# microsoft/fadtk

Measured on AMD Instinct MI355X. Metric: FAD scores/sec + cov-GEMM TFLOP/s (% MFMA peak), N=100k D=512, higher is better.
Workload: dtype f16 in, f16 MFMA with f32 accumulate over <= 8192-row runs, f64 across runs (moments); split-f16 MFMA iterations (f32 accumulate) + exact int8-MFMA products (int32 accumulate) + f64 correction (Frechet)

## Files before the change

fadtk_amd/_capi.py:

```python
from __future__ import annotations

import ctypes as C
import logging
import os
import threading
from pathlib import Path
from typing import Optional, Tuple

import numpy as np

log = logging.getLogger("fadtk_amd")

FAD_OK = 0
FAD_ERR_INVALID = -1
FAD_ERR_NO_DEVICE = -2
FAD_ERR_HIP = -3
FAD_ERR_ALLOC = -4
FAD_ERR_SHAPE = -5
FAD_ERR_TOO_FEW_ROWS = -6
FAD_ERR_NOT_FINITE = -7
FAD_ERR_NOT_CONVERGED = -8

FAD_F16, FAD_BF16, FAD_F32, FAD_F64 = 0, 1, 2, 3
FAD_KAD_GAUSSIAN, FAD_KAD_IQ, FAD_KAD_IMQ = 0, 1, 2
# ... 91 lines not shown
    "fad_moments_set_timing": (C.c_int, [_P, C.c_int]),
    "fad_moments_set_reference_mean": (C.c_int, [_P, C.c_int]),
    "fad_moments_last_timing": (C.c_int, [_P, C.POINTER(C.c_float), C.POINTER(C.c_float), C.POINTER(C.c_int)]),
    "fad_kad_last_plan": (C.c_int, [C.POINTER(_I64)]),
    "fad_stream_create_cu_mask": (C.c_int, [C.c_int, C.POINTER(C.c_uint32), C.c_int, C.POINTER(_P)]),
    "fad_stream_destroy": (C.c_int, [C.c_int, _P]),
    "fad_frechet": (C.c_int, [C.c_int, _P, _P, _P, _P, C.c_double, C.c_int, C.c_double, C.c_int, C.c_int, _P,
                              C.POINTER(C.c_double), C.POINTER(FadDiag)]),
    "fad_frechet_from_moments": (C.c_int, [_P, _P, C.c_int, C.c_double, C.c_int, C.c_double, C.c_int, _P,
                                           C.POINTER(C.c_double), C.POINTER(FadDiag)]),
    "fad_frechet_from_moments_begin": (C.c_int, [_P, _P, C.c_int, C.c_double, C.c_int, _P, C.POINTER(_P)]),
    "fad_frechet_end": (C.c_int, [_P, C.POINTER(C.c_double), C.POINTER(FadDiag)]),
    "fad_frechet_cancel": (C.c_int, [_P]),
    "fad_frechet_from_moments_multi_begin": (C.c_int, [C.c_int, C.POINTER(_P), C.POINTER(_P), C.c_int, C.c_double, C.c_int, _P, C.POINTER(_P)]),
    "fad_frechet_multi_end": (C.c_int, [_P, C.c_int, C.POINTER(C.c_double), C.POINTER(FadDiag)]),
    "fad_frechet_batched_vs_baseline": (C.c_int, [C.c_int, _P, _P, _P, _I64, _I64, C.c_int, C.POINTER(_I64), _I64,
                                                  C.c_int, C.c_int, C.c_int, _P, _P, _P]),
    "fad_resample_num_samples": (_I64, [_I64, C.c_int, C.c_int]),
    "fad_resample_kaiser": (C.c_int, [_P, _I64, C.c_int, C.c_int, C.c_int, _P, _I64, C.c_int, C.c_int, _P]),
    "fad_logmel_vggish_num_examples": (_I64, [_I64]),
    "fad_logmel_vggish": (C.c_int, [_P, C.POINTER(_I64), _I64, _P, _I64, C.POINTER(_I64), C.c_int, C.c_int, _P]),
    "fad_logmel_whisper": (C.c_int, [_P, C.POINTER(_I64), _I64, C.c_int, _P, C.c_int, C.c_int, _P]),
    "fad_logmel_htsat": (C.c_int, [_P, C.POINTER(_I64), _I64, _I64, _P, C.c_int, C.c_int, _P]),
    "fad_kad_median_distance": (C.c_int, [_P, _I64, _I64, _I64, C.c_int, C.c_int, C.POINTER(C.c_double), C.c_int, _P]),
    "fad_kad": (C.c_int, [_P, _I64, _I64, _P, _I64, _I64, _I64, C.c_int, C.c_int, C.c_double, C.POINTER(FadKadResult),
                          C.c_int, _P]),
    "fad_kad_individual": (C.c_int, [_P, _I64, _I64, _P, _I64, _I64, C.POINTER(_I64), _I64, _I64, C.c_int, C.c_int, C.c_double,
                                     C.POINTER(FadKadResult), _P, _P, _P, _P, C.c_int, _P]),
    "fad_kad_uncertainty": (C.c_int, [_P, _I64, _I64, C.POINTER(_P), C.POINTER(_I64), C.POINTER(_I64), C.c_int, _I64, C.c_int, C.c_int,
                                      C.c_double, C.POINTER(FadKadResult), _P, _P, _P, C.c_int, _P]),
# ... 162 lines not shown
```

fadtk_amd/csrc/frechet.hip:

```cpp
#include "frechet_internal.h"
#include "ns_mean.h"
#include "ns_fast.h"
#include "ns_fast_big.h"
#include "ns_fast_res.h"

#include <algorithm>
#include <atomic>
#include <cmath>
#include <type_traits>

namespace fad {

Pool& thread_pool(int device) {
    static thread_local PerThreadDevice<Pool> set;
    return set.get(device);
}
Workspace* free_slot(int device) {
    Pool& p = thread_pool(device);
    for (Workspace& w : p.slot)
        if (!w.busy) { w.pool = &p; return &w; }
    return nullptr;
}

SongKnobs SongKnobs::from_env() {
// ... 650 lines not shown
    const size_t dd = (size_t)d * d, nb = (size_t)d / 32;
    PairBlock b; size_t o = 0;
    auto take = [&](size_t bytes) { const size_t at = o; o += (bytes + 255) & ~(size_t)255; return at; };
    b.hdrA = take(sizeof(nsf::MatHdr)); b.hdrB = take(sizeof(nsf::MatHdr)); b.st = take(sizeof(NsState)); b.s32 = take(sizeof(Ns32State));
    b.partials = take(nb * nb * sizeof(double)); b.stats = take(nsf::kTileStats * nb * nb * sizeof(double));
    b.A64 = take(8 * dd); b.P = take(8 * dd);
    b.Y[0] = take(8 * dd); b.Y[1] = take(8 * dd); b.Z[0] = take(8 * dd); b.Z[1] = take(8 * dd); b.T = take(8 * dd);
    b.digA = take(6 * dd); b.digB = take(6 * dd);
    b.digY[0] = take(6 * dd); b.digYt[0] = take(6 * dd); b.digY[1] = take(6 * dd); b.digYt[1] = take(6 * dd);
    b.mus = take(2 * (size_t)d * sizeof(double)); b.covs = take(2 * dd * sizeof(double));
    b.Rv = take(8 * dd); b.Pv = take(8 * dd); b.Ev = take(8 * dd);
    b.stride = o;
    return b;
}

static int pairs_verify_enqueue(Workspace& ws, int d, int B, hipStream_t st) {
    const size_t dd = (size_t)d * d;
    const PairBlock L = pair_block(d);
    const size_t hs = song_host_stride(d);
    char* blk = static_cast<char*>(ws.fast_pairs.p);
    char* hpin = static_cast<char*>(ws.fast_pairs_pin);
    auto at = [&](size_t off) { return blk + off; };
    auto mat = [&](size_t off) { nsf::SplitMat m; m.a = reinterpret_cast<uint4*>(at(off)); m.at = reinterpret_cast<uint4*>(at(off + 4 * dd)); return m; };
    nsf::SplitArgs g;
    memset(&g, 0, sizeof(g));
    g.d = d; g.gen = ws.multi.gen; g.hA = reinterpret_cast<nsf::MatHdr*>(at(L.hdrA)); g.hB = reinterpret_cast<nsf::MatHdr*>(at(L.hdrB));
    g.pstride = (int64_t)L.stride; g.astride = (int64_t)L.stride;
    g.st = reinterpret_cast<NsState*>(at(L.st)); g.s32 = reinterpret_cast<Ns32State*>(at(L.s32));
    const nsf::SplitMat Y[2] = {mat(L.Y[0]), mat(L.Y[1])}, Z[2] = {mat(L.Z[0]), mat(L.Z[1])};
    const int nb = d / 32;
    int* h_words = reinterpret_cast<int*>(hpin + (nsf::kHostVals + (size_t)(nsf::kTileStats + 2) * nb * nb) * sizeof(double));
    double* h_vstats = reinterpret_cast<double*>(hpin + host_vstats_off(d));
    for (int b = 0; b < B; ++b) reinterpret_cast<int*>(reinterpret_cast<char*>(h_words) + (size_t)b * hs)[13] = 0;
    fast_verify_launch(d, (unsigned)B, g, Y, Z, mat(L.Rv), mat(L.Pv), mat(L.Ev), g.s32, h_vstats, h_words, (int64_t)hs, st);
    FAD_HIP_TRY(hipGetLastError());
    FAD_HIP_TRY(hipEventRecord(ws.done_ev, st));
    return FAD_OK;
}

static int pairs_enqueue(Workspace& ws, int d, int B, const fad_moments_t* const* h1, const fad_moments_t* const* h2, int ddof,
                         int mean_dtype, hipStream_t st) {
    const size_t dd = (size_t)d * d;
    const int nb = d / 32;
    constexpr int kPairsBigMin = 3;
    const bool big = B >= kPairsBigMin && d >= 256;
    const bool wide = wide_enabled(ws.pool);
    const int max_low = wide ? kMaxLowWide : kMaxLow;
    const int device = ws.job.device;
    const PairBlock L = pair_block(d);
    const size_t hs = song_host_stride(d);
    void* const before = ws.fast_pairs.p;
    FAD_TRY(ws.fast_pairs.reserve((size_t)(B > 16 ? kMaxMultiPairs : B > 8 ? 16 : B > 4 ? 8 : 4) * L.stride + 256));
    if (!ws.fast_pairs_pin || ws.fast_pairs_pin_cap < (size_t)B * hs) {
        if (ws.fast_pairs_pin) (void)hipHostFree(ws.fast_pairs_pin);
        ws.fast_pairs_pin = nullptr; ws.fast_pairs_pin_cap = 0;
        FAD_HIP_TRY(hipHostMalloc(&ws.fast_pairs_pin, (size_t)kMaxMultiPairs * hs + 4096, hipHostMallocDefault));
        ws.fast_pairs_pin_cap = (size_t)kMaxMultiPairs * hs + 4096;
    }
    char* blk = static_cast<char*>(ws.fast_pairs.p);
    char* hpin = static_cast<char*>(ws.fast_pairs_pin);
    double* h_vals = reinterpret_cast<double*>(hpin);
    double* h_stats = h_vals + nsf::kHostVals;
    int* h_words = reinterpret_cast<int*>(h_stats + (size_t)(nsf::kTileStats + 2) * nb * nb);
    auto at = [&](size_t off) { return blk + off; };
    auto mat = [&](size_t off) { nsf::SplitMat m; m.a = reinterpret_cast<uint4*>(at(off)); m.at = reinterpret_cast<uint4*>(at(off + 4 * dd)); return m; };
    const int gen = ++ws.fast_gen;
    if (ws.fast_gen > (1 << 30)) ws.fast_gen = 1;
    ws.multi.gen = gen;
    if (ws.fast_pairs.p != before) {
        FAD_HIP_TRY(hipMemset2DAsync(at(L.hdrA), L.stride, 0, sizeof(nsf::MatHdr), (size_t)B, st));
        FAD_HIP_TRY(hipMemset2DAsync(at(L.hdrB), L.stride, 0, sizeof(nsf::MatHdr), (size_t)B, st));
    }
    nsf::MatHdr* hA = reinterpret_cast<nsf::MatHdr*>(at(L.hdrA));
    nsf::MatHdr* hB = reinterpret_cast<nsf::MatHdr*>(at(L.hdrB));
    NsState* st0 = reinterpret_cast<NsState*>(at(L.st));
    Ns32State* s32_0 = reinterpret_cast<Ns32State*>(at(L.s32));
    double* partials = reinterpret_cast<double*>(at(L.partials));
    double* stats = reinterpret_cast<double*>(at(L.stats));
    double* A64 = reinterpret_cast<double*>(at(L.A64));
    const nsf::SplitMat P = mat(L.P), Y[2] = {mat(L.Y[0]), mat(L.Y[1])}, Z[2] = {mat(L.Z[0]), mat(L.Z[1])}, T = mat(L.T);
    uint4* digY[2] = {reinterpret_cast<uint4*>(at(L.digY[0])), reinterpret_cast<uint4*>(at(L.digY[1]))};
    uint4* digYt[2] = {reinterpret_cast<uint4*>(at(L.digYt[0])), reinterpret_cast<uint4*>(at(L.digYt[1]))};

    static_assert(2 * kMaxMultiPairs <= nsf::kPrepMaxSets, "PrepArgs holds two sets per pair of a batch");
    nsf::PrepArgs pa;
    memset(&pa, 0, sizeof(pa));
    for (int b = 0; b < B; ++b) {
        pa.accs[2 * b] = moments_packed(h1[b]); pa.accs[2 * b + 1] = moments_packed(h2[b]);
        pa.runs[2 * b] = moments_runsum(h1[b]); pa.runs[2 * b + 1] = moments_runsum(h2[b]);
    }
    pa.acc[0] = pa.accs[0]; pa.acc[1] = pa.accs[1];
    pa.d = d; pa.ddof = ddof; pa.gen = gen; pa.mean_dtype = mean_dtype;
    pa.mus = reinterpret_cast<double*>(at(L.mus)); pa.covs = reinterpret_cast<double*>(at(L.covs));
    pa.dig[0] = reinterpret_cast<uint4*>(at(L.digA)); pa.dig[1] = reinterpret_cast<uint4*>(at(L.digB));
    pa.st = st0; pa.hdr[0] = hA; pa.hdr[1] = hB;
    pa.batch = 2; pa.pstride = (int64_t)L.stride; pa.no_covs = 1;
    pa.per = ((dd / 2048) % 4 == 0) ? 4 : 2;
    hipLaunchKernelGGL(nsf::nsf_prepare, dim3((unsigned)(dd / 2048 / pa.per + 1), (unsigned)(2 * B)), dim3(512), 0, st, pa);

    auto split_args = [&]() {
        nsf::SplitArgs g;
        memset(&g, 0, sizeof(g));
        g.d = d; g.gen = gen; g.hA = hA; g.hB = hB; g.pstride = (int64_t)L.stride; g.astride = (int64_t)L.stride;
        g.st = st0; g.s32 = s32_0;
        if (wide) { g.scaled = 1; g.lp_wide = 1; g.l0_scale = kWideL0Scale; g.l0_min = kWideL0Min; }
        return g;
    };
    {
        nsf::I8Args a;
        memset(&a, 0, sizeof(a));
        a.Adig = reinterpret_cast<uint4*>(at(L.digA)); a.Bdig = reinterpret_cast<uint4*>(at(L.digB)); a.d = d; a.gen = gen; a.hA = hA; a.hB = hB;
        a.pstride = (int64_t)L.stride; a.astride = (int64_t)L.stride; a.stats = stats; a.A64 = A64; a.P = P; a.st = st0;
        if (big) FAD_TRY(fast_i8_big(d, nsf::I8_A, a, st, (unsigned)B, device));
        else fast_i8(d, nsf::I8_A, a, st, (unsigned)B);
        nsf::SplitArgs g = split_args();
        g.A[0] = P; g.B[0] = P; g.C[0] = Y[1]; g.C[1] = Z[1]; g.A64 = A64; g.statsA = stats;
        if (big) FAD_TRY(fast_split_big(d, nsf::SP_FIRST, g, st, (unsigned)B, device));
        else { g.Cdig[0] = digY[1]; g.Cdig_t[0] = digYt[1]; fast_split(d, nsf::SP_FIRST, g, st, (unsigned)B); }
    }
    int want = ws.pool ? ws.pool->lp_iters : 5;
    if (want < 2) want = 2;
    if (want > max_low) want = max_low;
    for (int k = 1; k < want; ++k) {
        const int cur = k & 1;
        nsf::SplitArgs g = split_args();
        g.A[0] = Z[cur]; g.B[0] = Y[cur]; g.C[0] = T; g.alpha = -0.5f; g.beta_eye = 1.5f; g.gamma = 1.0f;
        g.partials = partials; g.skip = &s32_0->done; g.k = k;
        if (big) FAD_TRY(fast_split_big(d, nsf::SP_T, g, st, (unsigned)B, device));
        else fast_split(d, nsf::SP_T, g, st, (unsigned)B);
        g = split_args();
        g.A[0] = Y[cur]; g.B[0] = T; g.C[0] = Y[cur ^ 1]; g.A[1] = T; g.B[1] = Z[cur]; g.C[1] = Z[cur ^ 1];
        if (!big) { g.Cdig[0] = digY[cur ^ 1]; g.Cdig_t[0] = digYt[cur ^ 1]; }
        g.skip = &s32_0->upd_skip[k & 1];
        g.k = k; g.max_low = max_low; g.nslots = big ? fast_big_t_slots(d, (unsigned)B) : nb * nb; g.chk_partials = partials; g.thr_pred = pred_threshold(ws.pool, d);
        if (big) FAD_TRY(fast_split_big(d, nsf::SP_U, g, st, (unsigned)B, device));
        else fast_split(d, nsf::SP_U, g, st, (unsigned)B);
    }
    if (big) {
        nsf::DigArgs dg;
        memset(&dg, 0, sizeof(dg));
        dg.d = d; dg.gen = gen; dg.hA = hA; dg.hB = hB; dg.pstride = (int64_t)L.stride; dg.astride = (int64_t)L.stride; dg.s32 = s32_0;
        dg.Y[0] = Y[0]; dg.Y[1] = Y[1]; dg.dig[0] = digY[0]; dg.dig[1] = digY[1]; dg.dig_t[0] = digYt[0]; dg.dig_t[1] = digYt[1];
        hipLaunchKernelGGL(nsf::nsf_digitize, dim3((unsigned)((dd / 16 + 255) / 256), 2, (unsigned)B), dim3(256), 0, st, dg);
    }
    {
        nsf::I8Args a;
        memset(&a, 0, sizeof(a));
        a.Adig = digY[0]; a.Bdig = digYt[0]; a.Adig_alt = digY[1]; a.Bdig_alt = digYt[1]; a.sel = &s32_0->final_iter;
        a.d = d; a.gen = gen; a.hA = hA; a.hB = hB; a.pstride = (int64_t)L.stride; a.astride = (int64_t)L.stride; a.hstride = (int64_t)hs;
        a.skip = &s32_0->skip_corr; a.stats = h_stats; a.st = st0; a.A64in = A64;
        a.Y[0] = Y[0]; a.Y[1] = Y[1]; a.Z[0] = Z[0]; a.Z[1] = Z[1]; a.s32 = s32_0; a.host_words = h_words; a.host_vals = h_vals;
        if (wide) { a.Rv = mat(L.Rv); a.scaled = 1; }
        for (int b = 0; b < B; ++b) { int* w = reinterpret_cast<int*>(reinterpret_cast<char*>(h_words) + (size_t)b * hs); w[12] = 0; w[13] = 0; }
        if (big) FAD_TRY(fast_i8_big(d, nsf::I8_G, a, st, (unsigned)B, device));
        else fast_i8(d, nsf::I8_G, a, st, (unsigned)B);
    }
    FAD_HIP_TRY(hipGetLastError());
    if (!ws.done_ev) FAD_HIP_TRY(hipEventCreateWithFlags(&ws.done_ev, hipEventDisableTiming));
    if (wide && ws.pool && ws.pool->lp_verify) return pairs_verify_enqueue(ws, d, B, st);
    FAD_HIP_TRY(hipEventRecord(ws.done_ev, st));
    return FAD_OK;
}

static int mixed_begin(const NsProblem& pb, int device, hipStream_t stream, Workspace& ws) {
    const int d = pb.d;
    const int64_t dd = (int64_t)d * d;
    FAD_TRY(ws.mats.reserve((size_t)(6 * dd) * sizeof(double)));
    FAD_TRY(ws.mats32.reserve((size_t)(5 * dd) * sizeof(float)));
    const size_t hbytes = ws.job.fast ? fast_pinned_bytes(d) : sizeof(NsState) + sizeof(MixedResult);
    if (!ws.pinned || ws.pinned_cap < hbytes) {
        if (ws.pinned) (void)hipHostFree(ws.pinned);
        ws.pinned = nullptr; ws.pinned_cap = 0;
        FAD_HIP_TRY(hipHostMalloc(&ws.pinned, hbytes + 4096, hipHostMallocDefault));
        ws.pinned_cap = hbytes + 4096;
// ... 257 lines not shown
    }
    DeviceGuard g(device);
    hipStream_t st = static_cast<hipStream_t>(stream);
    Workspace* wsp = free_slot(device);
    if (!wsp) return set_error(FAD_ERR_INVALID, "all %d Frechet slots of this thread are in flight: collect one with fad_frechet_end", Pool::kSlots);
    Workspace& ws = *wsp;
    ws.pool = &thread_pool(device);
    ws.job = Workspace::Job();
    ws.job.d = d; ws.job.device = device; ws.job.stream = st; ws.job.eps = eps; ws.job.mean_dtype = mean_dtype; ws.job.ddof = ddof;
    ws.multi = Workspace::Multi();
    ws.multi.count = count;
    for (int b = 0; b < count; ++b) { ws.multi.h1[b] = h1[b]; ws.multi.h2[b] = h2[b]; }
    if (fast_eligible(ws, d, 0, 0.0)) {
        for (int b = 0; b < count; ++b) { FAD_TRY(moments_settle(h1[b], st)); FAD_TRY(moments_settle(h2[b], st)); }
        FAD_TRY(pairs_enqueue(ws, d, count, h1, h2, ddof, mean_dtype, st));
        for (int b = 0; b < count; ++b) { FAD_TRY(moments_mark_read(h1[b], st)); FAD_TRY(moments_mark_read(h2[b], st)); }
        ws.multi.enqueued = true;
    }
    ws.busy = true;
    *job = reinterpret_cast<fad_frechet_job_t*>(wsp);
    return FAD_OK;
}

int fad_frechet_multi_end(fad_frechet_job_t* job, int count, double* out_fad, fad_diag_t* diag) {
    if (!job || !out_fad) return set_error(FAD_ERR_INVALID, "NULL argument");
    Workspace& ws = *reinterpret_cast<Workspace*>(job);
    if (!ws.busy) return set_error(FAD_ERR_INVALID, "this job was collected already");
    if (count != ws.multi.count) return set_error(FAD_ERR_INVALID, "this job holds %d pairs, not %d", ws.multi.count, count);
    const Workspace::Job j = ws.job;
    const Workspace::Multi m = ws.multi;
    DeviceGuard g(j.device);
// ... 66 lines not shown
            NsState* hst = nullptr;
            if (r2 == FAD_OK) {
                NsState* dstates = static_cast<NsState*>(ws.small.p);
                enqueue_clear_states(dstates, count, j.stream);
                uint32_t mask = 0;
                for (int b = 0; b < count; ++b) if (done[b] || chain_status[b] != 2) mask |= (1u << b);
                if (mask) enqueue_mark_states_done(dstates, mask, count, j.stream);
                nsf::PrepArgs pc;
                memset(&pc, 0, sizeof(pc));
                for (int b = 0; b < count; ++b) { pc.accs[2 * b] = moments_packed(m.h1[b]); pc.accs[2 * b + 1] = moments_packed(m.h2[b]); }
                pc.d = d; pc.ddof = j.ddof; pc.batch = 2; pc.pstride = (int64_t)L.stride;
                pc.covs = reinterpret_cast<double*>(blk + L.covs);
                hipLaunchKernelGGL(nsf::nsf_pairs_covs, dim3((unsigned)(dd / 2048), (unsigned)(2 * count)), dim3(512), 0, j.stream, pc);
                NsProblem pb{d, count, covs, stride, covs + dd, stride, mus, stride, mus + d, stride, j.mean_dtype};
                r2 = run_ns(pb, 0, 0.0, j.device, j.stream, ws, &hst, false, nullptr, (ws.pool && ws.pool->f64_iters_multi > 0) ? ws.pool->f64_iters_multi + 1 : 0);
            }
            if (r2 == FAD_OK && hst) {
                int most = 0;
                for (int b = 0; b < count; ++b) {
                    if (done[b] || chain_status[b] != 2) continue;
                    const NsState& q = hst[b];
                    if (q.nonfinite || q.conv == 0 || !q.finished || q.final_iter < 0) continue;
                    const double tr_sqrt = sqrt(q.c) * q.tr_last;
                    out_fad[b] = q.mean_term + q.tr1 + q.tr2 - 2.0 * tr_sqrt;
                    if (diag) {
                        fad_diag_t& g2 = diag[b];
                        memset(&g2, 0, sizeof(g2));
                        g2.iters = q.final_iter + 1; g2.converged = q.conv; g2.used_eps = 0; g2.route = 0; g2.residual = q.res_last;
                        g2.scale = q.c; g2.mean_term = q.mean_term; g2.tr1 = q.tr1; g2.tr2 = q.tr2; g2.tr_sqrt = tr_sqrt;
                    }
// ... 2 lines not shown
                }
                if (most > 0 && ws.pool) ws.pool->f64_iters_multi = most;
            }
        }
    }
    ws.busy = false;
    ws.multi = Workspace::Multi();
    for (int b = 0; b < count; ++b) {
        if (done[b]) continue;
        const int r1 = fad_frechet_from_moments(m.h1[b], m.h2[b], j.ddof, j.eps, 0, 0.0, j.mean_dtype, j.stream, &out_fad[b], diag ? &diag[b] : nullptr);
        if (r1 != FAD_OK && rc == FAD_OK) rc = r1;
    }
    return rc;
}

int fad_frechet_cancel(fad_frechet_job_t* job) {
    if (!job) return set_error(FAD_ERR_INVALID, "NULL argument");
    Workspace& ws = *reinterpret_cast<Workspace*>(job);
    if (!ws.busy) return FAD_OK;
    DeviceGuard g(ws.job.device);
    if ((ws.job.mixed || ws.multi.enqueued) && ws.done_ev) FAD_HIP_TRY(hipEventSynchronize(ws.done_ev));
    else FAD_HIP_TRY(hipStreamSynchronize(ws.job.stream));
    ws.busy = false;
    ws.job = Workspace::Job();
    ws.multi = Workspace::Multi();
    return FAD_OK;
}

}
```

fadtk_amd/csrc/frechet_internal.h:

```cpp
#pragma once
#include "fad_common.h"
#include "ns_check.h"
#include "ns32.h"

#include <cstdlib>
#include <vector>

struct fad_moments;
namespace fad {
const double* moments_packed(const fad_moments* h);
int moments_settle(const fad_moments* h, hipStream_t st);
int moments_mark_read(const fad_moments* h, hipStream_t st);
int moments_device(const fad_moments* h);
int moments_dim(const fad_moments* h);
const float* moments_runsum(const fad_moments* h);

constexpr int kStatScal = 8;
static inline int64_t stat_blocks(int d) { return cdiv(d, 32); }
static inline size_t stat_doubles(int d) { const int64_t nb = stat_blocks(d); return (size_t)(2 * nb * d + kStatScal * nb * nb); }

constexpr int kMaxMultiPairs = 32;

struct Workspace : NsWorkspace {
    DevBuf rows, offs, songbuf, songmat, rows2, songrun, songjobs;
    DevBuf base_root;
    void* song_pin = nullptr; size_t song_pin_cap = 0;
    DevBuf mats32;
    DevBuf fast;
    int fast_gen = 0;
    DevBuf songcov;
    DevBuf fast_songs;
    void* fast_songs_pin = nullptr; size_t fast_songs_pin_cap = 0;
    DevBuf fast_pairs;
    void* fast_pairs_pin = nullptr; size_t fast_pairs_pin_cap = 0;
    struct Multi {
        int count = 0, gen = 0;
        bool enqueued = false;
        const fad_moments_t* h1[kMaxMultiPairs] = {nullptr}; const fad_moments_t* h2[kMaxMultiPairs] = {nullptr};
    } multi;
    bool busy = false;
    struct Job {
        int d = 0, device = 0, k = 0, mean_dtype = -1, ddof = 1;
        bool mixed = false;
        bool fast = false;
        int gen = 0;
        double eps = 0.0;
        hipStream_t stream = nullptr;
        const double *cov1 = nullptr, *cov2 = nullptr, *mu1 = nullptr, *mu2 = nullptr;
    } job;
    hipEvent_t done_ev = nullptr;
    struct Pool* pool = nullptr;
    void release_all() {
        release(); rows.release(); offs.release(); songbuf.release(); songmat.release(); rows2.release(); songrun.release(); songjobs.release(); mats32.release(); base_root.release(); fast.release();
        fast_songs.release(); songcov.release(); fast_pairs.release();
        if (fast_pairs_pin) { (void)hipHostFree(fast_pairs_pin); fast_pairs_pin = nullptr; fast_pairs_pin_cap = 0; }
        if (fast_songs_pin) { (void)hipHostFree(fast_songs_pin); fast_songs_pin = nullptr; fast_songs_pin_cap = 0; }
        if (done_ev) { (void)hipEventDestroy(done_ev); done_ev = nullptr; }
        if (song_pin) { (void)hipHostFree(song_pin); song_pin = nullptr; song_pin_cap = 0; }
    }
    int reserve_song_pin(size_t bytes) {
        if (song_pin && song_pin_cap >= bytes) return FAD_OK;
        if (song_pin) (void)hipHostFree(song_pin);
        song_pin = nullptr; song_pin_cap = 0;
        FAD_HIP_TRY(hipHostMalloc(&song_pin, bytes + bytes / 2 + 4096, hipHostMallocDefault));
        song_pin_cap = bytes + bytes / 2 + 4096;
        return FAD_OK;
    }
};


struct Pool {
    static constexpr int kSlots = 8;
    Workspace slot[kSlots];
    int lp_iters = 5;
    bool lp_hopeless = false;
    bool lp_verify = false;
    int lp_wide = -1;
    int f64_iters = 0;
    int f64_iters_multi = 0;
    int mixed = -1;
    int fast = -1;
    double pred_thr = 0.0;
    void release_all() { for (Workspace& w : slot) w.release_all(); }
};
Pool& thread_pool(int device);
Workspace* free_slot(int device);

struct NsProblem {
    int d; int64_t B;
    const double* cov1; int64_t s_cov1;
    const double* cov2; int64_t s_cov2;
    const double* mu1; int64_t s_mu1;
    const double* mu2; int64_t s_mu2;
    int mean_dtype;
    int sym = 0;
};

static inline int ns_pstride(int d) {
// ... 49 lines not shown
```

fadtk_amd/hip.py:

```python
from __future__ import annotations

import ctypes as C
from typing import Optional, Sequence, Tuple

import numpy as np

from . import _capi as K


class Moments:

    def __init__(self, d: int, device: int = 0):
        self._lib = K.load_library()
        K.require_gpu(device)
        self.d = int(d)
        self.device = int(device)
        h = C.c_void_p()
        K.check(self._lib.fad_moments_create(self.d, self.device, C.byref(h)), "fad_moments_create")
        self._h = h

    def close(self):
        if getattr(self, "_h", None):
            self._lib.fad_moments_destroy(self._h)
            self._h = None
# ... 332 lines not shown
        self._lds = (C.c_int64 * m)(*[max(v[3], a.d) for a, v in zip(accs, views)])
        self._lib = accs[0]._lib

    def run(self, reset: bool = False) -> None:
        st = self._accs[0]._stream()
        if reset:
            K.check(self._lib.fad_moments_reset_multi(self._m, self._hs, st), "fad_moments_reset_multi")
        K.check(self._lib.fad_moments_update_multi(self._m, self._hs, self._ptrs, self._ns, self._lds, self._code, st), "fad_moments_update_multi")
        for a, k in zip(self._accs, self._keep):
            a._keep = k


class FrechetMultiJob:

    MAX_PAIRS = 32

    def __init__(self, pairs, ddof: int = 1, eps: float = 1e-6, mean_dtype: int = -1):
        import threading
        self._lib = K.load_library()
        self._owner = threading.get_ident()
        self._n = len(pairs)
        if not 1 <= self._n <= self.MAX_PAIRS:
            raise ValueError(f"a FrechetMultiJob holds 1..{self.MAX_PAIRS} pairs")
        a = (C.c_void_p * self._n)(*[p[0]._h for p in pairs])
        b = (C.c_void_p * self._n)(*[p[1]._h for p in pairs])
        job = C.c_void_p()
        K.check(self._lib.fad_frechet_from_moments_multi_begin(self._n, a, b, int(ddof), float(eps), int(mean_dtype),
                                                               K.current_stream_ptr(pairs[0][0].device), C.byref(job)),
                "fad_frechet_from_moments_multi_begin")
        self._job = job
# ... 21 lines not shown
        job, self._job = self._job, None
        K.check(self._lib.fad_frechet_multi_end(job, self._n, out.ctypes.data_as(C.POINTER(C.c_double)), diag), "fad_frechet_multi_end")
        return out, diag

    def cancel(self):
        import threading
        if self._job is not None and threading.get_ident() == self._owner:
            job, self._job = self._job, None
            K.check(self._lib.fad_frechet_cancel(job), "fad_frechet_cancel")

    def __del__(self):
        try:
            self.cancel()
        except Exception:
            pass


def frechet_batched(mu_b, cov_b, rows, offsets: Sequence[int], mean_mode: int = 1, device: int = 0):
    lib = K.load_library()
    K.require_gpu(device)
    base_on_dev = K._is_torch(mu_b) and K._is_torch(cov_b) and mu_b.is_cuda and cov_b.is_cuda
    if base_on_dev:
        import torch
        mu_t = mu_b.to(torch.float64).contiguous(); cov_t = cov_b.to(torch.float64).contiguous()
        d = int(mu_t.shape[0])
        assert tuple(cov_t.shape) == (d, d)
    else:
        mu_b = K.f64_host(mu_b)
        d = mu_b.shape[0]
        cov_b = K.f64_host(cov_b, (d, d))
# ... 577 lines not shown
```

include/fad_hip.h:

```cpp
#ifndef FAD_HIP_H
#define FAD_HIP_H

#include <stdint.h>

#ifdef __cplusplus
extern "C" {
#endif

#define FAD_ABI_VERSION 2

typedef enum fad_status {
    FAD_OK = 0,
    FAD_ERR_INVALID = -1,
    FAD_ERR_NO_DEVICE = -2,
    FAD_ERR_HIP = -3,
    FAD_ERR_ALLOC = -4,
    FAD_ERR_SHAPE = -5,
    FAD_ERR_TOO_FEW_ROWS = -6,
    FAD_ERR_NOT_FINITE = -7,
    FAD_ERR_NOT_CONVERGED = -8
} fad_status;

typedef enum fad_dtype { FAD_F16 = 0, FAD_BF16 = 1, FAD_F32 = 2, FAD_F64 = 3 } fad_dtype;

// ... 69 lines not shown

#define FAD_MEAN_SECOND_ONLY 16
int fad_frechet_from_moments(const fad_moments_t* h1, const fad_moments_t* h2, int ddof, double eps,
                             int max_iter, double tol, int mean_dtype, void* stream, double* out_fad, fad_diag_t* diag);

typedef struct fad_frechet_job fad_frechet_job_t;
int fad_frechet_from_moments_begin(const fad_moments_t* h1, const fad_moments_t* h2, int ddof, double eps, int mean_dtype,
                                   void* stream, fad_frechet_job_t** job);
int fad_frechet_end(fad_frechet_job_t* job, double* out_fad, fad_diag_t* diag);
int fad_frechet_cancel(fad_frechet_job_t* job);

#define FAD_MULTI_MAX_PAIRS 32
int fad_frechet_from_moments_multi_begin(int count, const fad_moments_t* const* h1, const fad_moments_t* const* h2, int ddof,
                                         double eps, int mean_dtype, void* stream, fad_frechet_job_t** job);
int fad_frechet_multi_end(fad_frechet_job_t* job, int count, double* out_fad, fad_diag_t* diag);

int fad_frechet_batched_vs_baseline(int d, const double* mu_b, const double* cov_b,
                                    const void* rows, int64_t n_rows, int64_t ld, int dtype,
                                    const int64_t* offsets, int64_t n_songs, int mean_mode,
                                    int on_device, int device, void* stream,
                                    double* out_scores, int32_t* out_status);

int64_t fad_logmel_vggish_num_examples(int64_t n_samples);
int fad_logmel_vggish(const float* wav, const int64_t* offsets, int64_t n_clips, float* out,
                      int64_t out_capacity_examples, int64_t* example_offsets, int on_device, int device,
                      void* stream);
int fad_logmel_whisper(const float* wav, const int64_t* offsets, int64_t n_clips, int n_mels, float* out,
                       int on_device, int device, void* stream);
int fad_logmel_htsat(const float* wav, const int64_t* offsets, int64_t n_clips, int64_t n_frames_out,
                     float* out, int on_device, int device, void* stream);
// ... 113 lines not shown
```

Before: 12030.

## Split large multi-pair Frechet batches across two streams for concurrent execution

When a multi-pair Frechet batch holds 16 or more pairs, it is now split into two halves. The second half's prepare, int8, split-iteration, digitize and final kernels run on a side stream that forks from and joins back to the main stream. Launches are interleaved per stage so the two halves can overlap on the GPU, filling CUs that a single batched launch leaves idle. It also adds a counter for f64 fallback batches and exposes it through the C API and Python. The cost is extra stream and event management, plus moments reads marked on the side stream.

```diff
diff --git a/fadtk_amd/_capi.py b/fadtk_amd/_capi.py
--- a/fadtk_amd/_capi.py
+++ b/fadtk_amd/_capi.py
@@ -129,6 +129,7 @@
     "fad_frechet_cancel": (C.c_int, [_P]),
     "fad_frechet_from_moments_multi_begin": (C.c_int, [C.c_int, C.POINTER(_P), C.POINTER(_P), C.c_int, C.c_double, C.c_int, _P, C.POINTER(_P)]),
     "fad_frechet_multi_end": (C.c_int, [_P, C.c_int, C.POINTER(C.c_double), C.POINTER(FadDiag)]),
+    "fad_frechet_multi_f64_batches": (C.c_longlong, [C.c_int]),
     "fad_frechet_batched_vs_baseline": (C.c_int, [C.c_int, _P, _P, _P, _I64, _I64, C.c_int, C.POINTER(_I64), _I64,
                                                   C.c_int, C.c_int, C.c_int, _P, _P, _P]),
     "fad_resample_num_samples": (_I64, [_I64, C.c_int, C.c_int]),
diff --git a/fadtk_amd/csrc/frechet.hip b/fadtk_amd/csrc/frechet.hip
--- a/fadtk_amd/csrc/frechet.hip
+++ b/fadtk_amd/csrc/frechet.hip
@@ -688,12 +688,12 @@
     return b;
 }
 
-static int pairs_verify_enqueue(Workspace& ws, int d, int B, hipStream_t st) {
+static int pairs_verify_launch(Workspace& ws, int d, int b0, int B, hipStream_t st) {
     const size_t dd = (size_t)d * d;
     const PairBlock L = pair_block(d);
     const size_t hs = song_host_stride(d);
-    char* blk = static_cast<char*>(ws.fast_pairs.p);
-    char* hpin = static_cast<char*>(ws.fast_pairs_pin);
+    char* blk = static_cast<char*>(ws.fast_pairs.p) + (size_t)b0 * L.stride;
+    char* hpin = static_cast<char*>(ws.fast_pairs_pin) + (size_t)b0 * hs;
     auto at = [&](size_t off) { return blk + off; };
     auto mat = [&](size_t off) { nsf::SplitMat m; m.a = reinterpret_cast<uint4*>(at(off)); m.at = reinterpret_cast<uint4*>(at(off + 4 * dd)); return m; };
     nsf::SplitArgs g;
@@ -708,130 +708,192 @@
     for (int b = 0; b < B; ++b) reinterpret_cast<int*>(reinterpret_cast<char*>(h_words) + (size_t)b * hs)[13] = 0;
     fast_verify_launch(d, (unsigned)B, g, Y, Z, mat(L.Rv), mat(L.Pv), mat(L.Ev), g.s32, h_vstats, h_words, (int64_t)hs, st);
     FAD_HIP_TRY(hipGetLastError());
+    return FAD_OK;
+}
+static int pairs_verify_enqueue(Workspace& ws, int d, int B, hipStream_t st) {
+    FAD_TRY(pairs_verify_launch(ws, d, 0, B, st));
     FAD_HIP_TRY(hipEventRecord(ws.done_ev, st));
     return FAD_OK;
 }
 
-static int pairs_enqueue(Workspace& ws, int d, int B, const fad_moments_t* const* h1, const fad_moments_t* const* h2, int ddof,
-                         int mean_dtype, hipStream_t st) {
+struct PairsRun { int b0, B; hipStream_t st; };
+
+static int pairs_launches(Workspace& ws, int d, const PairsRun* run, int nruns, const fad_moments_t* const* h1, const fad_moments_t* const* h2,
+                          int ddof, int mean_dtype, int gen) {
     const size_t dd = (size_t)d * d;
     const int nb = d / 32;
     constexpr int kPairsBigMin = 3;
-    const bool big = B >= kPairsBigMin && d >= 256;
     const bool wide = wide_enabled(ws.pool);
     const int max_low = wide ? kMaxLowWide : kMaxLow;
     const int device = ws.job.device;
     const PairBlock L = pair_block(d);
     const size_t hs = song_host_stride(d);
-    void* const before = ws.fast_pairs.p;
-    FAD_TRY(ws.fast_pairs.reserve((size_t)(B > 16 ? kMaxMultiPairs : B > 8 ? 16 : B > 4 ? 8 : 4) * L.stride + 256));
-    if (!ws.fast_pairs_pin || ws.fast_pairs_pin_cap < (size_t)B * hs) {
-        if (ws.fast_pairs_pin) (void)hipHostFree(ws.fast_pairs_pin);
-        ws.fast_pairs_pin = nullptr; ws.fast_pairs_pin_cap = 0;
-        FAD_HIP_TRY(hipHostMalloc(&ws.fast_pairs_pin, (size_t)kMaxMultiPairs * hs + 4096, hipHostMallocDefault));
-        ws.fast_pairs_pin_cap = (size_t)kMaxMultiPairs * hs + 4096;
-    }
-    char* blk = static_cast<char*>(ws.fast_pairs.p);
-    char* hpin = static_cast<char*>(ws.fast_pairs_pin);
-    double* h_vals = reinterpret_cast<double*>(hpin);
-    double* h_stats = h_vals + nsf::kHostVals;
-    int* h_words = reinterpret_cast<int*>(h_stats + (size_t)(nsf::kTileStats + 2) * nb * nb);
-    auto at = [&](size_t off) { return blk + off; };
-    auto mat = [&](size_t off) { nsf::SplitMat m; m.a = reinterpret_cast<uint4*>(at(off)); m.at = reinterpret_cast<uint4*>(at(off + 4 * dd)); return m; };
-    const int gen = ++ws.fast_gen;
-    if (ws.fast_gen > (1 << 30)) ws.fast_gen = 1;
-    ws.multi.gen = gen;
-    if (ws.fast_pairs.p != before) {
-        FAD_HIP_TRY(hipMemset2DAsync(at(L.hdrA), L.stride, 0, sizeof(nsf::MatHdr), (size_t)B, st));
-        FAD_HIP_TRY(hipMemset2DAsync(at(L.hdrB), L.stride, 0, sizeof(nsf::MatHdr), (size_t)B, st));
-    }
-    nsf::MatHdr* hA = reinterpret_cast<nsf::MatHdr*>(at(L.hdrA));
-    nsf::MatHdr* hB = reinterpret_cast<nsf::MatHdr*>(at(L.hdrB));
-    NsState* st0 = reinterpret_cast<NsState*>(at(L.st));
-    Ns32State* s32_0 = reinterpret_cast<Ns32State*>(at(L.s32));
-    double* partials = reinterpret_cast<double*>(at(L.partials));
-    double* stats = reinterpret_cast<double*>(at(L.stats));
-    double* A64 = reinterpret_cast<double*>(at(L.A64));
-    const nsf::SplitMat P = mat(L.P), Y[2] = {mat(L.Y[0]), mat(L.Y[1])}, Z[2] = {mat(L.Z[0]), mat(L.Z[1])}, T = mat(L.T);
-    uint4* digY[2] = {reinterpret_cast<uint4*>(at(L.digY[0])), reinterpret_cast<uint4*>(at(L.digY[1]))};
-    uint4* digYt[2] = {reinterpret_cast<uint4*>(at(L.digYt[0])), reinterpret_cast<uint4*>(at(L.digYt[1]))};
+    struct Ptrs {
+        bool big;
+        nsf::MatHdr *hA, *hB; NsState* st0; Ns32State* s32_0;
+        double *partials, *stats, *A64, *mus, *covs, *h_vals, *h_stats;
+        int* h_words;
+        nsf::SplitMat P, Y[2], Z[2], T, Rv;
+        uint4 *digA, *digB, *digY[2], *digYt[2];
+    } ptrs[2];
+    for (int r = 0; r < nruns; ++r) {
+        char* blk = static_cast<char*>(ws.fast_pairs.p) + (size_t)run[r].b0 * L.stride;
+        char* hpin = static_cast<char*>(ws.fast_pairs_pin) + (size_t)run[r].b0 * hs;
+        auto at = [&](size_t off) { return blk + off; };
+        auto mat = [&](size_t off) { nsf::SplitMat m; m.a = reinterpret_cast<uint4*>(at(off)); m.at = reinterpret_cast<uint4*>(at(off + 4 * dd)); return m; };
+        Ptrs& p = ptrs[r];
+        p.big = run[r].B >= kPairsBigMin && d >= 256;
+        p.hA = reinterpret_cast<nsf::MatHdr*>(at(L.hdrA)); p.hB = reinterpret_cast<nsf::MatHdr*>(at(L.hdrB));
+        p.st0 = reinterpret_cast<NsState*>(at(L.st)); p.s32_0 = reinterpret_cast<Ns32State*>(at(L.s32));
+        p.partials = reinterpret_cast<double*>(at(L.partials)); p.stats = reinterpret_cast<double*>(at(L.stats));
+        p.A64 = reinterpret_cast<double*>(at(L.A64));
+        p.mus = reinterpret_cast<double*>(at(L.mus)); p.covs = reinterpret_cast<double*>(at(L.covs));
+        p.P = mat(L.P); p.Y[0] = mat(L.Y[0]); p.Y[1] = mat(L.Y[1]); p.Z[0] = mat(L.Z[0]); p.Z[1] = mat(L.Z[1]); p.T = mat(L.T); p.Rv = mat(L.Rv);
+        p.digA = reinterpret_cast<uint4*>(at(L.digA)); p.digB = reinterpret_cast<uint4*>(at(L.digB));
+        p.digY[0] = reinterpret_cast<uint4*>(at(L.digY[0])); p.digY[1] = reinterpret_cast<uint4*>(at(L.digY[1]));
+        p.digYt[0] = reinterpret_cast<uint4*>(at(L.digYt[0])); p.digYt[1] = reinterpret_cast<uint4*>(at(L.digYt[1]));
+        p.h_vals = reinterpret_cast<double*>(hpin);
+        p.h_stats = p.h_vals + nsf::kHostVals;
+        p.h_words = reinterpret_cast<int*>(p.h_stats + (size_t)(nsf::kTileStats + 2) * nb * nb);
+    }
 
     static_assert(2 * kMaxMultiPairs <= nsf::kPrepMaxSets, "PrepArgs holds two sets per pair of a batch");
-    nsf::PrepArgs pa;
-    memset(&pa, 0, sizeof(pa));
-    for (int b = 0; b < B; ++b) {
-        pa.accs[2 * b] = moments_packed(h1[b]); pa.accs[2 * b + 1] = moments_packed(h2[b]);
-        pa.runs[2 * b] = moments_runsum(h1[b]); pa.runs[2 * b + 1] = moments_runsum(h2[b]);
-    }
-    pa.acc[0] = pa.accs[0]; pa.acc[1] = pa.accs[1];
-    pa.d = d; pa.ddof = ddof; pa.gen = gen; pa.mean_dtype = mean_dtype;
-    pa.mus = reinterpret_cast<double*>(at(L.mus)); pa.covs = reinterpret_cast<double*>(at(L.covs));
-    pa.dig[0] = reinterpret_cast<uint4*>(at(L.digA)); pa.dig[1] = reinterpret_cast<uint4*>(at(L.digB));
-    pa.st = st0; pa.hdr[0] = hA; pa.hdr[1] = hB;
-    pa.batch = 2; pa.pstride = (int64_t)L.stride; pa.no_covs = 1;
-    pa.per = ((dd / 2048) % 4 == 0) ? 4 : 2;
-    hipLaunchKernelGGL(nsf::nsf_prepare, dim3((unsigned)(dd / 2048 / pa.per + 1), (unsigned)(2 * B)), dim3(512), 0, st, pa);
-
-    auto split_args = [&]() {
+    for (int r = 0; r < nruns; ++r) {
+        const Ptrs& p = ptrs[r]; const int B = run[r].B, b0 = run[r].b0;
+        nsf::PrepArgs pa;
+        memset(&pa, 0, sizeof(pa));
+        for (int b = 0; b < B; ++b) {
+            pa.accs[2 * b] = moments_packed(h1[b0 + b]); pa.accs[2 * b + 1] = moments_packed(h2[b0 + b]);
+            pa.runs[2 * b] = moments_runsum(h1[b0 + b]); pa.runs[2 * b + 1] = moments_runsum(h2[b0 + b]);
+        }
+        pa.acc[0] = pa.accs[0]; pa.acc[1] = pa.accs[1];
+        pa.d = d; pa.ddof = ddof; pa.gen = gen; pa.mean_dtype = mean_dtype;
+        pa.mus = p.mus; pa.covs = p.covs;
+        pa.dig[0] = p.digA; pa.dig[1] = p.digB;
+        pa.st = p.st0; pa.hdr[0] = p.hA; pa.hdr[1] = p.hB;
+        pa.batch = 2; pa.pstride = (int64_t)L.stride; pa.no_covs = 1;
+        pa.per = ((dd / 2048) % 4 == 0) ? 4 : 2;
+        hipLaunchKernelGGL(nsf::nsf_prepare, dim3((unsigned)(dd / 2048 / pa.per + 1), (unsigned)(2 * B)), dim3(512), 0, run[r].st, pa);
+    }
+
+    auto split_args = [&](const Ptrs& p) {
         nsf::SplitArgs g;
         memset(&g, 0, sizeof(g));
-        g.d = d; g.gen = gen; g.hA = hA; g.hB = hB; g.pstride = (int64_t)L.stride; g.astride = (int64_t)L.stride;
-        g.st = st0; g.s32 = s32_0;
+        g.d = d; g.gen = gen; g.hA = p.hA; g.hB = p.hB; g.pstride = (int64_t)L.stride; g.astride = (int64_t)L.stride;
+        g.st = p.st0; g.s32 = p.s32_0;
         if (wide) { g.scaled = 1; g.lp_wide = 1; g.l0_scale = kWideL0Scale; g.l0_min = kWideL0Min; }
         return g;
     };
-    {
+    for (int r = 0; r < nruns; ++r) {
+        const Ptrs& p = ptrs[r]; const unsigned B = (unsigned)run[r].B; hipStream_t st = run[r].st;
         nsf::I8Args a;
         memset(&a, 0, sizeof(a));
-        a.Adig = reinterpret_cast<uint4*>(at(L.digA)); a.Bdig = reinterpret_cast<uint4*>(at(L.digB)); a.d = d; a.gen = gen; a.hA = hA; a.hB = hB;
-        a.pstride = (int64_t)L.stride; a.astride = (int64_t)L.stride; a.stats = stats; a.A64 = A64; a.P = P; a.st = st0;
-        if (big) FAD_TRY(fast_i8_big(d, nsf::I8_A, a, st, (unsigned)B, device));
-        else fast_i8(d, nsf::I8_A, a, st, (unsigned)B);
-        nsf::SplitArgs g = split_args();
-        g.A[0] = P; g.B[0] = P; g.C[0] = Y[1]; g.C[1] = Z[1]; g.A64 = A64; g.statsA = stats;
-        if (big) FAD_TRY(fast_split_big(d, nsf::SP_FIRST, g, st, (unsigned)B, device));
-        else { g.Cdig[0] = digY[1]; g.Cdig_t[0] = digYt[1]; fast_split(d, nsf::SP_FIRST, g, st, (unsigned)B); }
+        a.Adig = p.digA; a.Bdig = p.digB; a.d = d; a.gen = gen; a.hA = p.hA; a.hB = p.hB;
+        a.pstride = (int64_t)L.stride; a.astride = (int64_t)L.stride; a.stats = p.stats; a.A64 = p.A64; a.P = p.P; a.st = p.st0;
+        if (p.big) FAD_TRY(fast_i8_big(d, nsf::I8_A, a, st, B, device));
+        else fast_i8(d, nsf::I8_A, a, st, B);
+    }
+    for (int r = 0; r < nruns; ++r) {
+        const Ptrs& p = ptrs[r]; const unsigned B = (unsigned)run[r].B; hipStream_t st = run[r].st;
+        nsf::SplitArgs g = split_args(p);
+        g.A[0] = p.P; g.B[0] = p.P; g.C[0] = p.Y[1]; g.C[1] = p.Z[1]; g.A64 = p.A64; g.statsA = p.stats;
+        if (p.big) FAD_TRY(fast_split_big(d, nsf::SP_FIRST, g, st, B, device));
+        else { g.Cdig[0] = p.digY[1]; g.Cdig_t[0] = p.digYt[1]; fast_split(d, nsf::SP_FIRST, g, st, B); }
     }
     int want = ws.pool ? ws.pool->lp_iters : 5;
     if (want < 2) want = 2;
     if (want > max_low) want = max_low;
     for (int k = 1; k < want; ++k) {
         const int cur = k & 1;
-        nsf::SplitArgs g = split_args();
-        g.A[0] = Z[cur]; g.B[0] = Y[cur]; g.C[0] = T; g.alpha = -0.5f; g.beta_eye = 1.5f; g.gamma = 1.0f;
-        g.partials = partials; g.skip = &s32_0->done; g.k = k;
-        if (big) FAD_TRY(fast_split_big(d, nsf::SP_T, g, st, (unsigned)B, device));
-        else fast_split(d, nsf::SP_T, g, st, (unsigned)B);
-        g = split_args();
-        g.A[0] = Y[cur]; g.B[0] = T; g.C[0] = Y[cur ^ 1]; g.A[1] = T; g.B[1] = Z[cur]; g.C[1] = Z[cur ^ 1];
-        if (!big) { g.Cdig[0] = digY[cur ^ 1]; g.Cdig_t[0] = digYt[cur ^ 1]; }
-        g.skip = &s32_0->upd_skip[k & 1];
-        g.k = k; g.max_low = max_low; g.nslots = big ? fast_big_t_slots(d, (unsigned)B) : nb * nb; g.chk_partials = partials; g.thr_pred = pred_threshold(ws.pool, d);
-        if (big) FAD_TRY(fast_split_big(d, nsf::SP_U, g, st, (unsigned)B, device));
-        else fast_split(d, nsf::SP_U, g, st, (unsigned)B);
-    }
-    if (big) {
+        for (int r = 0; r < nruns; ++r) {
+            const Ptrs& p = ptrs[r]; const unsigned B = (unsigned)run[r].B; hipStream_t st = run[r].st;
+            nsf::SplitArgs g = split_args(p);
+            g.A[0] = p.Z[cur]; g.B[0] = p.Y[cur]; g.C[0] = p.T; g.alpha = -0.5f; g.beta_eye = 1.5f; g.gamma = 1.0f;
+            g.partials = p.partials; g.skip = &p.s32_0->done; g.k = k;
+            if (p.big) FAD_TRY(fast_split_big(d, nsf::SP_T, g, st, B, device));
+            else fast_split(d, nsf::SP_T, g, st, B);
+        }
+        for (int r = 0; r < nruns; ++r) {
+            const Ptrs& p = ptrs[r]; const unsigned B = (unsigned)run[r].B; hipStream_t st = run[r].st;
+            nsf::SplitArgs g = split_args(p);
+            g.A[0] = p.Y[cur]; g.B[0] = p.T; g.C[0] = p.Y[cur ^ 1]; g.A[1] = p.T; g.B[1] = p.Z[cur]; g.C[1] = p.Z[cur ^ 1];
+            if (!p.big) { g.Cdig[0] = p.digY[cur ^ 1]; g.Cdig_t[0] = p.digYt[cur ^ 1]; }
+            g.skip = &p.s32_0->upd_skip[k & 1];
+            g.k = k; g.max_low = max_low; g.nslots = p.big ? fast_big_t_slots(d, B) : nb * nb; g.chk_partials = p.partials; g.thr_pred = pred_threshold(ws.pool, d);
+            if (p.big) FAD_TRY(fast_split_big(d, nsf::SP_U, g, st, B, device));
+            else fast_split(d, nsf::SP_U, g, st, B);
+        }
+    }
+    for (int r = 0; r < nruns; ++r) {
+        const Ptrs& p = ptrs[r]; const unsigned B = (unsigned)run[r].B;
+        if (!p.big) continue;
         nsf::DigArgs dg;
         memset(&dg, 0, sizeof(dg));
-        dg.d = d; dg.gen = gen; dg.hA = hA; dg.hB = hB; dg.pstride = (int64_t)L.stride; dg.astride = (int64_t)L.stride; dg.s32 = s32_0;
-        dg.Y[0] = Y[0]; dg.Y[1] = Y[1]; dg.dig[0] = digY[0]; dg.dig[1] = digY[1]; dg.dig_t[0] = digYt[0]; dg.dig_t[1] = digYt[1];
-        hipLaunchKernelGGL(nsf::nsf_digitize, dim3((unsigned)((dd / 16 + 255) / 256), 2, (unsigned)B), dim3(256), 0, st, dg);
-    }
-    {
+        dg.d = d; dg.gen = gen; dg.hA = p.hA; dg.hB = p.hB; dg.pstride = (int64_t)L.stride; dg.astride = (int64_t)L.stride; dg.s32 = p.s32_0;
+        dg.Y[0] = p.Y[0]; dg.Y[1] = p.Y[1]; dg.dig[0] = p.digY[0]; dg.dig[1] = p.digY[1]; dg.dig_t[0] = p.digYt[0]; dg.dig_t[1] = p.digYt[1];
+        hipLaunchKernelGGL(nsf::nsf_digitize, dim3((unsigned)((dd / 16 + 255) / 256), 2, B), dim3(256), 0, run[r].st, dg);
+    }
+    for (int r = 0; r < nruns; ++r) {
+        const Ptrs& p = ptrs[r]; const unsigned B = (unsigned)run[r].B; hipStream_t st = run[r].st;
         nsf::I8Args a;
         memset(&a, 0, sizeof(a));
-        a.Adig = digY[0]; a.Bdig = digYt[0]; a.Adig_alt = digY[1]; a.Bdig_alt = digYt[1]; a.sel = &s32_0->final_iter;
-        a.d = d; a.gen = gen; a.hA = hA; a.hB = hB; a.pstride = (int64_t)L.stride; a.astride = (int64_t)L.stride; a.hstride = (int64_t)hs;
-        a.skip = &s32_0->skip_corr; a.stats = h_stats; a.st = st0; a.A64in = A64;
-        a.Y[0] = Y[0]; a.Y[1] = Y[1]; a.Z[0] = Z[0]; a.Z[1] = Z[1]; a.s32 = s32_0; a.host_words = h_words; a.host_vals = h_vals;
-        if (wide) { a.Rv = mat(L.Rv); a.scaled = 1; }
-        for (int b = 0; b < B; ++b) { int* w = reinterpret_cast<int*>(reinterpret_cast<char*>(h_words) + (size_t)b * hs); w[12] = 0; w[13] = 0; }
-        if (big) FAD_TRY(fast_i8_big(d, nsf::I8_G, a, st, (unsigned)B, device));
-        else fast_i8(d, nsf::I8_G, a, st, (unsigned)B);
+        a.Adig = p.digY[0]; a.Bdig = p.digYt[0]; a.Adig_alt = p.digY[1]; a.Bdig_alt = p.digYt[1]; a.sel = &p.s32_0->final_iter;
+        a.d = d; a.gen = gen; a.hA = p.hA; a.hB = p.hB; a.pstride = (int64_t)L.stride; a.astride = (int64_t)L.stride; a.hstride = (int64_t)hs;
+        a.skip = &p.s32_0->skip_corr; a.stats = p.h_stats; a.st = p.st0; a.A64in = p.A64;
+        a.Y[0] = p.Y[0]; a.Y[1] = p.Y[1]; a.Z[0] = p.Z[0]; a.Z[1] = p.Z[1]; a.s32 = p.s32_0; a.host_words = p.h_words; a.host_vals = p.h_vals;
+        if (wide) { a.Rv = p.Rv; a.scaled = 1; }
+        for (unsigned b = 0; b < B; ++b) { int* w = reinterpret_cast<int*>(reinterpret_cast<char*>(p.h_words) + (size_t)b * hs); w[12] = 0; w[13] = 0; }
+        if (p.big) FAD_TRY(fast_i8_big(d, nsf::I8_G, a, st, B, device));
+        else fast_i8(d, nsf::I8_G, a, st, B);
     }
     FAD_HIP_TRY(hipGetLastError());
+    if (wide && ws.pool && ws.pool->lp_verify)
+        for (int r = 0; r < nruns; ++r) FAD_TRY(pairs_verify_launch(ws, d, run[r].b0, run[r].B, run[r].st));
+    return FAD_OK;
+}
+
+static int pairs_enqueue(Workspace& ws, int d, int count, const fad_moments_t* const* h1, const fad_moments_t* const* h2, int ddof,
+                         int mean_dtype, hipStream_t st) {
+    const PairBlock L = pair_block(d);
+    const size_t hs = song_host_stride(d);
+    void* const before = ws.fast_pairs.p;
+    FAD_TRY(ws.fast_pairs.reserve((size_t)(count > 16 ? kMaxMultiPairs : count > 8 ? 16 : count > 4 ? 8 : 4) * L.stride + 256));
+    if (!ws.fast_pairs_pin || ws.fast_pairs_pin_cap < (size_t)count * hs) {
+        if (ws.fast_pairs_pin) (void)hipHostFree(ws.fast_pairs_pin);
+        ws.fast_pairs_pin = nullptr; ws.fast_pairs_pin_cap = 0;
+        FAD_HIP_TRY(hipHostMalloc(&ws.fast_pairs_pin, (size_t)kMaxMultiPairs * hs + 4096, hipHostMallocDefault));
+        ws.fast_pairs_pin_cap = (size_t)kMaxMultiPairs * hs + 4096;
+    }
+    const int gen = ++ws.fast_gen;
+    if (ws.fast_gen > (1 << 30)) ws.fast_gen = 1;
+    ws.multi.gen = gen;
+    if (ws.fast_pairs.p != before) {
+        char* blk = static_cast<char*>(ws.fast_pairs.p);
+        FAD_HIP_TRY(hipMemset2DAsync(blk + L.hdrA, L.stride, 0, sizeof(nsf::MatHdr), (size_t)count, st));
+        FAD_HIP_TRY(hipMemset2DAsync(blk + L.hdrB, L.stride, 0, sizeof(nsf::MatHdr), (size_t)count, st));
+    }
     if (!ws.done_ev) FAD_HIP_TRY(hipEventCreateWithFlags(&ws.done_ev, hipEventDisableTiming));
-    if (wide && ws.pool && ws.pool->lp_verify) return pairs_verify_enqueue(ws, d, B, st);
+
+    PairsRun run[2] = {{0, count, st}, {0, 0, nullptr}};
+    int nruns = 1;
+    const int n1 = multi_first_run(count);
+    if (n1 < count && ws.pool) {
+        Pool& pool = *ws.pool;
+        if (!pool.side) FAD_HIP_TRY(hipStreamCreateWithFlags(&pool.side, hipStreamNonBlocking));
+        if (!ws.fork_ev) FAD_HIP_TRY(hipEventCreateWithFlags(&ws.fork_ev, hipEventDisableTiming));
+        if (!ws.join_ev) FAD_HIP_TRY(hipEventCreateWithFlags(&ws.join_ev, hipEventDisableTiming));
+        FAD_HIP_TRY(hipEventRecord(ws.fork_ev, st));
+        FAD_HIP_TRY(hipStreamWaitEvent(pool.side, ws.fork_ev, 0));
+        run[0].B = n1; run[1] = PairsRun{n1, count - n1, pool.side};
+        nruns = 2;
+    }
+    int rc = pairs_launches(ws, d, run, nruns, h1, h2, ddof, mean_dtype, gen);
+    if (nruns == 2) {
+        hipError_t e = hipEventRecord(ws.join_ev, run[1].st);
+        if (e == hipSuccess) e = hipStreamWaitEvent(st, ws.join_ev, 0);
+        if (e != hipSuccess && rc == FAD_OK) rc = set_error(FAD_ERR_HIP, "joining the side stream failed: %s", hipGetErrorString(e));
+    }
+    if (rc != FAD_OK) return rc;
     FAD_HIP_TRY(hipEventRecord(ws.done_ev, st));
     return FAD_OK;
 }
@@ -1119,7 +1181,11 @@
     if (fast_eligible(ws, d, 0, 0.0)) {
         for (int b = 0; b < count; ++b) { FAD_TRY(moments_settle(h1[b], st)); FAD_TRY(moments_settle(h2[b], st)); }
         FAD_TRY(pairs_enqueue(ws, d, count, h1, h2, ddof, mean_dtype, st));
-        for (int b = 0; b < count; ++b) { FAD_TRY(moments_mark_read(h1[b], st)); FAD_TRY(moments_mark_read(h2[b], st)); }
+        const int n1 = (multi_first_run(count) < count && ws.pool->side) ? multi_first_run(count) : count;
+        for (int b = 0; b < count; ++b) {
+            hipStream_t reader = b < n1 ? st : ws.pool->side;
+            FAD_TRY(moments_mark_read(h1[b], reader)); FAD_TRY(moments_mark_read(h2[b], reader));
+        }
         ws.multi.enqueued = true;
     }
     ws.busy = true;
@@ -1216,6 +1282,7 @@
                 hipLaunchKernelGGL(nsf::nsf_pairs_covs, dim3((unsigned)(dd / 2048), (unsigned)(2 * count)), dim3(512), 0, j.stream, pc);
                 NsProblem pb{d, count, covs, stride, covs + dd, stride, mus, stride, mus + d, stride, j.mean_dtype};
                 r2 = run_ns(pb, 0, 0.0, j.device, j.stream, ws, &hst, false, nullptr, (ws.pool && ws.pool->f64_iters_multi > 0) ? ws.pool->f64_iters_multi + 1 : 0);
+                if (ws.pool) ++ws.pool->f64_batches;
             }
             if (r2 == FAD_OK && hst) {
                 int most = 0;
@@ -1248,6 +1315,8 @@
     return rc;
 }
 
+long long fad_frechet_multi_f64_batches(int device) { return device < 0 ? 0 : thread_pool(device).f64_batches; }
+
 int fad_frechet_cancel(fad_frechet_job_t* job) {
     if (!job) return set_error(FAD_ERR_INVALID, "NULL argument");
     Workspace& ws = *reinterpret_cast<Workspace*>(job);
diff --git a/fadtk_amd/csrc/frechet_internal.h b/fadtk_amd/csrc/frechet_internal.h
--- a/fadtk_amd/csrc/frechet_internal.h
+++ b/fadtk_amd/csrc/frechet_internal.h
@@ -20,6 +20,8 @@
 static inline size_t stat_doubles(int d) { const int64_t nb = stat_blocks(d); return (size_t)(2 * nb * d + kStatScal * nb * nb); }
 
 constexpr int kMaxMultiPairs = 32;
+constexpr int kMultiSplitMin = 16;
+constexpr int multi_first_run(int n) { return n >= kMultiSplitMin ? (n + 1) / 2 : n; }
 
 struct Workspace : NsWorkspace {
     DevBuf rows, offs, songbuf, songmat, rows2, songrun, songjobs;
@@ -49,6 +51,7 @@
         const double *cov1 = nullptr, *cov2 = nullptr, *mu1 = nullptr, *mu2 = nullptr;
     } job;
     hipEvent_t done_ev = nullptr;
+    hipEvent_t fork_ev = nullptr, join_ev = nullptr;
     struct Pool* pool = nullptr;
     void release_all() {
         release(); rows.release(); offs.release(); songbuf.release(); songmat.release(); rows2.release(); songrun.release(); songjobs.release(); mats32.release(); base_root.release(); fast.release();
@@ -56,6 +59,8 @@
         if (fast_pairs_pin) { (void)hipHostFree(fast_pairs_pin); fast_pairs_pin = nullptr; fast_pairs_pin_cap = 0; }
         if (fast_songs_pin) { (void)hipHostFree(fast_songs_pin); fast_songs_pin = nullptr; fast_songs_pin_cap = 0; }
         if (done_ev) { (void)hipEventDestroy(done_ev); done_ev = nullptr; }
+        if (fork_ev) { (void)hipEventDestroy(fork_ev); fork_ev = nullptr; }
+        if (join_ev) { (void)hipEventDestroy(join_ev); join_ev = nullptr; }
         if (song_pin) { (void)hipHostFree(song_pin); song_pin = nullptr; song_pin_cap = 0; }
     }
     int reserve_song_pin(size_t bytes) {
@@ -81,7 +86,12 @@
     int mixed = -1;
     int fast = -1;
     double pred_thr = 0.0;
-    void release_all() { for (Workspace& w : slot) w.release_all(); }
+    hipStream_t side = nullptr;
+    long long f64_batches = 0;
+    void release_all() {
+        for (Workspace& w : slot) w.release_all();
+        if (side) { (void)hipStreamDestroy(side); side = nullptr; }
+    }
 };
 Pool& thread_pool(int device);
 Workspace* free_slot(int device);
diff --git a/fadtk_amd/hip.py b/fadtk_amd/hip.py
--- a/fadtk_amd/hip.py
+++ b/fadtk_amd/hip.py
@@ -370,6 +370,7 @@
 class FrechetMultiJob:
 
     MAX_PAIRS = 32
+    SPLIT_MIN = 16
 
     def __init__(self, pairs, ddof: int = 1, eps: float = 1e-6, mean_dtype: int = -1):
         import threading
@@ -421,6 +422,10 @@
             self.cancel()
         except Exception:
             pass
+
+
+def frechet_multi_f64_batches(device: int = 0) -> int:
+    return int(K.load_library().fad_frechet_multi_f64_batches(int(device)))
 
 
 def frechet_batched(mu_b, cov_b, rows, offsets: Sequence[int], mean_mode: int = 1, device: int = 0):
diff --git a/include/fad_hip.h b/include/fad_hip.h
--- a/include/fad_hip.h
+++ b/include/fad_hip.h
@@ -107,6 +107,7 @@
 int fad_frechet_from_moments_multi_begin(int count, const fad_moments_t* const* h1, const fad_moments_t* const* h2, int ddof,
                                          double eps, int mean_dtype, void* stream, fad_frechet_job_t** job);
 int fad_frechet_multi_end(fad_frechet_job_t* job, int count, double* out_fad, fad_diag_t* diag);
+long long fad_frechet_multi_f64_batches(int device);
 
 int fad_frechet_batched_vs_baseline(int d, const double* mu_b, const double* cov_b,
                                     const void* rows, int64_t n_rows, int64_t ld, int dtype,
```

Measured after the change: 11840. 0.984x the previous value.
